# ooowedyn/InkLayer

Measured on AMD Instinct MI355X. Metric: sketches/sec end-to-end (GroundingDINO+SAM) at 1024x1024, higher is better.
Workload: dtype f16 (MFMA, f32 accumulate; f32 residual/norm/softmax; split-f16 = fp32-grade operands for patch-embed, neck, mask decoder); 1 GPU; full GroundingDINO Swin-T + SAM ViT-H pipeline, batch=8 per GPU, 1024x1024 synthetic sketches, 16 boxes/sketch, random-init weights; global_batch=8, parallelism=image-parallel x1

## Files before the change

include/inklayer_hip.h:

```cpp
#ifndef INKLAYER_HIP_H
#define INKLAYER_HIP_H

#include <stdint.h>

#ifdef __cplusplus
extern "C" {
#endif

#define INK_ABI_VERSION 8
int ink_abi_version(void);

typedef struct InkGemm {
  const void* A;
  const void* W;
  const float* bias;
  const float* col_scale;
  const float* residual;
  const int32_t* row_map;
  void* C;
  int32_t M, N, K;
  int32_t lda, ldw, ldr, ldc;
  int32_t act;
  int32_t c_f16;
} InkGemm;
// ... 119 lines not shown
                     int64_t ldo, void* stream);

int ink_attn_fewq(const void* Q, int64_t ldq, const void* K, int64_t ldk, const void* V, int64_t ldv,
                  int32_t n_batch, int32_t n_q, int32_t n_k, int32_t n_heads, int32_t head_dim, float scale,
                  const int32_t* q_batch_rows, const int32_t* kv_batch_rows, const float* k_add, void* O, int64_t ldo,
                  void* stream);

int ink_biattn_colstats(const float* scores, int32_t B, int32_t S, int32_t HT, float* part_ws, float* stats, void* stream);

int ink_fusion_fold_workspace(int32_t B, int32_t S, int64_t* out_floats);
int ink_fusion_fold(float* v_f32, int32_t B, int32_t S, const float* lnv_g, const float* lnv_b, float eps,
                    const float* text_k_f32, const float* text_vl_f32, int64_t ld_text, int32_t T, const void* Wq_f16,
                    const float* bq, const void* Wvv_f16, const float* bvv, const void* Wo_f16, const float* bo,
                    const float* gamma_v, float scale, float* ws, void* out_l_f16, const float* pos, void* out16_pos,
                    void* out16, void* stream);

int ink_sam_upscale_pack(const void* ws_f16, void* blob_f16, void* stream);
int ink_sam_upscale_tail(const float* u0, int64_t ld_tok, int32_t n, int32_t g, const float* ln_g, const float* ln_b, float eps,
                         const void* blob_f16, const float* b3, const float* hyper, int32_t n_masks, float* low,
                         void* stream);

int ink_proj256_ln_pack(const void* ws_f16, void* blob_f16, void* stream);
int ink_proj256_ln(const float* a_f32, const void* blob_f16, const float* bias, const float* res_f32,
                   const int32_t* res_batch_rows, int32_t rows_per_batch, const float* ln_g, const float* ln_b, float eps,
                   int64_t rows, float* out_f32, void* out_split_f16, void* stream);

int ink_ffn256_pack_bytes(int32_t hid, int32_t with_pre, int64_t* out_bytes);
int ink_ffn256_pack(const void* w1_f16, const float* b1, const void* w2_f16, int32_t hid, const void* wpre_f16, void* blob,
                    void* stream);
int ink_ffn256_fused(const void* x_f16, int64_t ldx, const float* res_f32, const void* blob, const float* b2,
                     const float* ln_g, const float* ln_b, float eps, int32_t M, int32_t hid, const float* pre_bias,
                     const float* pre_ln_g, const float* pre_ln_b, float* out_f32, void* stream);

int ink_topk_rowmax(const float* logits, int32_t B, int32_t S, int32_t T, int32_t K, int32_t* out_idx,
                    float* out_val, void* cand_ws, void* stream);

int ink_sine_embed4(const float* ref, const float* dim_t, int32_t N, void* out_f16, void* stream);

int ink_box_refine(const float* delta, int64_t ldd, const float* ref, int32_t N, int32_t ref_is_logit,
                   float* out, void* stream);

int ink_mask_cleanup_workspace_ints(int32_t n, int32_t H, int32_t W, int32_t k, int64_t* out_ints);
int ink_mask_cleanup(const void* masks_u8, int32_t n, int32_t H, int32_t W, int32_t k, int32_t area_threshold,
                     double aspect_threshold, void* tmp_a_u8, void* tmp_b_u8, int32_t* workspace, void* out_u8,
                     void* stream);

int ink_mask_sketch_iou_counts(const void* masks_u8, const void* sketch_rgb_u8, int32_t n, int32_t H, int32_t W,
                               void* bits_ws_u64, int32_t* counts, void* stream);

int ink_sam_amg_stats(const float* low, int32_t n, const int32_t* index, int32_t m, const int32_t* m_dev, int32_t S,
                      int32_t L, int32_t in_h, int32_t in_w, int32_t crop_h, int32_t crop_w, double thr, double offset,
                      int32_t x0, int32_t y0, int32_t orig_h, int32_t orig_w, int32_t* table, void* planes_u64,
                      float* out_logits, void* stream);

int ink_mask_rle_counts(const void* planes_u64, const int32_t* select, int32_t k, int32_t H, int32_t W,
                        int32_t* n_counts, void* stream);
int ink_mask_rle_write(const void* planes_u64, const int32_t* select, int32_t k, int32_t H, int32_t W,
                       const int32_t* offsets, int32_t* counts, void* stream);

int ink_mask_small_regions_workspace_ints(int32_t k, int32_t H, int32_t W, int64_t* out_ints);
int ink_mask_small_regions(const void* planes_u64, int32_t k, int32_t H, int32_t W, int32_t min_area, int32_t holes,
                           void* tmp_planes_u64, int32_t* workspace, void* out_planes_u64, int32_t* changed, void* stream);

int ink_box_nms(const float* boxes, const float* scores, int32_t n, float iou_threshold, void* workspace_u64,
                int32_t* keep, int32_t* n_keep, void* stream);

// ... 114 lines not shown
```

inklayer_amd/_lib.py:

```python
from __future__ import annotations

import ctypes as C
import os
from pathlib import Path

_LIB_PATH = Path(__file__).resolve().parent / "lib" / "libinklayer_hip.so"
_lib = None

c_void_p, c_int, c_i64, c_float = C.c_void_p, C.c_int32, C.c_int64, C.c_float


class InkGemm(C.Structure):
    _fields_ = [
        ("A", c_void_p), ("W", c_void_p), ("bias", c_void_p), ("col_scale", c_void_p),
        ("residual", c_void_p), ("row_map", c_void_p), ("C", c_void_p),
        ("M", c_int), ("N", c_int), ("K", c_int),
        ("lda", c_int), ("ldw", c_int), ("ldr", c_int), ("ldc", c_int),
        ("act", c_int), ("c_f16", c_int),
    ]


class InkAttn(C.Structure):
    _fields_ = [
        ("Q", c_void_p), ("K", c_void_p), ("V", c_void_p), ("O", c_void_p),
# ... 40 lines not shown
                               c_void_p],
    "ink_box_nms": [c_void_p, c_void_p, c_int, c_float, c_void_p, c_void_p, c_void_p, c_void_p],
    "ink_ms_deform_attn_forward": [c_void_p, C.POINTER(c_i64), C.POINTER(c_i64), c_void_p, c_void_p, c_int,
                                   c_int, c_int, c_int, c_int, c_int, c_int, c_int, c_void_p, c_void_p],
    "ink_ms_deform_attn_forward_dev": [c_void_p, c_void_p, c_void_p, c_void_p, c_void_p, c_int, c_int, c_int, c_int,
                                       c_int, c_int, c_int, c_int, c_int, c_void_p, c_void_p],
    "ink_ms_deform_attn_backward_dev": [c_void_p, c_void_p, c_void_p, c_void_p, c_void_p, c_void_p, c_int, c_int, c_int,
                                        c_int, c_int, c_int, c_int, c_int, c_int, c_void_p, c_void_p, c_void_p,
                                        c_void_p],
    "ink_msda_fused": [c_void_p, c_void_p, c_i64, c_void_p, c_int, c_i64, c_i64, C.POINTER(c_int), c_int,
                       c_int, c_int, c_void_p, c_void_p],
    "ink_swin_patchify": [c_void_p, c_int, c_int, C.POINTER(c_float), C.POINTER(c_float), c_void_p, c_void_p],
    "ink_layernorm_merge4": [c_void_p, c_i64, c_void_p, c_void_p, c_float, c_void_p, c_int, c_int, c_void_p,
                             c_void_p],
    "ink_groupnorm_nhwc": [c_void_p, c_int, c_int, c_int, c_int, c_void_p, c_void_p, c_float, c_void_p,
                           c_void_p, c_i64, c_void_p],
    "ink_gather_rows": [c_void_p, c_i64, c_i64, c_void_p, c_i64, c_int, c_int, c_int, c_void_p, c_void_p,
                        c_void_p],
    "ink_biattn_fusion": [c_void_p, c_void_p, c_int, c_int, c_int, c_int, c_float, c_void_p, c_void_p,
                          c_void_p, c_int, c_void_p, c_void_p, c_void_p],
    "ink_biattn_colstats": [c_void_p, c_int, c_int, c_int, c_void_p, c_void_p, c_void_p],
    "ink_fusion_fold_workspace": [c_int, c_int, C.POINTER(c_i64)],
    "ink_relpos_bias64_f16": [c_void_p, c_i64, c_void_p, c_void_p, c_int, c_int, c_int, c_float, c_void_p, c_void_p, c_void_p],
    "ink_proj256_ln_pack": [c_void_p, c_void_p, c_void_p],
    "ink_proj256_ln": [c_void_p, c_void_p, c_void_p, c_void_p, c_void_p, c_int, c_void_p, c_void_p, c_float, c_i64, c_void_p,
                       c_void_p, c_void_p],
    "ink_sam_upscale_pack": [c_void_p, c_void_p, c_void_p],
    "ink_sam_upscale_tail": [c_void_p, c_i64, c_int, c_int, c_void_p, c_void_p, c_float, c_void_p, c_void_p, c_void_p,
                             c_int, c_void_p, c_void_p],
    "ink_ffn256_pack_bytes": [c_int, c_int, C.POINTER(c_i64)],
    "ink_ffn256_pack": [c_void_p, c_void_p, c_void_p, c_int, c_void_p, c_void_p, c_void_p],
    "ink_ffn256_fused": [c_void_p, c_i64, c_void_p, c_void_p, c_void_p, c_void_p, c_void_p, c_float, c_int, c_int,
                         c_void_p, c_void_p, c_void_p, c_void_p, c_void_p],
    "ink_fusion_fold": [c_void_p, c_int, c_int, c_void_p, c_void_p, c_float, c_void_p, c_void_p, c_i64, c_int, c_void_p,
                        c_void_p, c_void_p, c_void_p, c_void_p, c_void_p, c_void_p, c_float, c_void_p, c_void_p, c_void_p,
                        c_void_p, c_void_p, c_void_p],
    "ink_attn_fewkeys": [c_void_p, c_i64, c_void_p, c_i64, c_void_p, c_i64, c_int, c_int, c_int, c_int, c_int,
                         c_float, c_void_p, c_void_p, c_void_p, c_int, c_void_p, c_i64, c_void_p],
    "ink_attn_fewq": [c_void_p, c_i64, c_void_p, c_i64, c_void_p, c_i64, c_int, c_int, c_int, c_int, c_int,
                      c_float, c_void_p, c_void_p, c_void_p, c_void_p, c_i64, c_void_p],
    "ink_topk_rowmax": [c_void_p, c_int, c_int, c_int, c_int, c_void_p, c_void_p, c_void_p, c_void_p],
    "ink_sine_embed4": [c_void_p, c_void_p, c_int, c_void_p, c_void_p],
    "ink_box_refine": [c_void_p, c_i64, c_void_p, c_int, c_int, c_void_p, c_void_p],
    "ink_mask_cleanup_workspace_ints": [c_int, c_int, c_int, c_int, C.POINTER(c_i64)],
    "ink_mask_cleanup": [c_void_p, c_int, c_int, c_int, c_int, c_int, C.c_double, c_void_p, c_void_p, c_void_p,
                         c_void_p, c_void_p],
    "ink_mask_sketch_iou_counts": [c_void_p, c_void_p, c_int, c_int, c_int, c_void_p, c_void_p, c_void_p],
    "ink_refine_sketch_planes": [c_void_p, c_int, c_int, c_void_p, c_void_p, c_void_p],
    "ink_bitplane_pack": [c_void_p, c_int, c_int, c_int, c_int, c_void_p, c_void_p],
    "ink_refine_depth_samples": [c_void_p, c_int, c_void_p, c_void_p, c_int, c_int, c_int, c_void_p, c_void_p, c_void_p],
    "ink_refine_pair_tables": [c_void_p, c_void_p, c_int, c_int, c_int, c_void_p, c_void_p, c_void_p, c_void_p,
                               c_void_p, c_void_p],
    "ink_refine_composite": [c_void_p, c_void_p, c_int, c_int, c_int, c_void_p, c_void_p, c_void_p],
    "ink_refine_relabel_clean": [c_void_p, c_void_p, c_int, c_int, c_void_p, c_void_p],
    "ink_refine_grow_workspace": [c_int, c_int, C.POINTER(c_i64), C.POINTER(c_i64)],
    "ink_refine_grow": [c_void_p, c_void_p, c_int, c_int, c_void_p, c_void_p, c_void_p, c_void_p, c_void_p, c_void_p,
                        c_int, c_void_p, c_void_p],
    "ink_refine_query_dists": [c_void_p, c_void_p, c_void_p, c_int, c_int, c_int, c_void_p, c_void_p],
    "ink_refine_finalize": [c_void_p, c_void_p, c_int, c_void_p, c_int, c_int, c_void_p, c_void_p, c_void_p, c_void_p],
    "ink_host_sparse_sample": [c_void_p, c_int, c_int, c_void_p, c_int, c_void_p],
    "ink_host_assign_unlabeled": [c_void_p, c_int, c_void_p, c_int, c_void_p, c_void_p, c_void_p, c_int, c_void_p],
    "ink_depth_patchify": [c_void_p, c_int, c_int, c_int, c_int, c_int, c_int, C.POINTER(C.c_double), C.POINTER(C.c_double),
                           c_int, c_void_p, c_void_p],
    "ink_resize_bilinear_ac_nhwc": [c_void_p, c_int, c_int, c_int, c_int, c_int, c_int, c_void_p, c_void_p, c_void_p],
    "ink_im2col3x3_ex_f16": [c_void_p, c_int, c_int, c_int, c_int, c_int, c_int, c_void_p, c_void_p],
    "ink_layers_otsu_planes": [c_void_p, c_int, c_int, c_int, c_int, c_void_p, c_void_p, c_void_p, c_void_p],
# ... 64 lines not shown
```

inklayer_amd/build.py:

```python
from __future__ import annotations

import os
import subprocess
import sys
from concurrent.futures import ThreadPoolExecutor
from pathlib import Path

ROOT = Path(__file__).resolve().parent
CSRC = ROOT / "csrc"
LIBDIR = ROOT / "lib"
OBJDIR = LIBDIR / "obj"
LIB = LIBDIR / "libinklayer_hip.so"
HIPCC = os.environ.get("HIPCC", "/opt/rocm/bin/hipcc")
FLAGS = ["--offload-arch=gfx950", "-O3", "-std=c++17", "-fPIC", "-ffp-contract=off",
         "-mllvm", "-amdgpu-mfma-vgpr-form",

         "-Wall", "-Wno-unused-function", "-Wno-unused-variable"]


def _newest_header() -> float:
    hs = list(CSRC.glob("*.h")) + list((ROOT.parent / "include").glob("*.h"))
    return max(h.stat().st_mtime for h in hs)


NO_SPILL = {"ffn_fused.hip", "proj_ln.hip", "amg.hip", "layers.hip", "inpaint_ops.hip", "visualize.hip"}


def _check_no_spill(src: Path, remarks: str) -> None:
    name = None
    for line in remarks.splitlines():
        if "Function Name:" in line:
            name = line.split("Function Name:")[1].split("[")[0].strip()
        elif "ScratchSize [bytes/lane]:" in line:
            n = int(line.split("ScratchSize [bytes/lane]:")[1].split("[")[0])
            if n != 0:
                raise RuntimeError(f"{src.name}: kernel {name} spills ({n} bytes of scratch per lane) - the kernels of "
                                   f"this file must stay in registers (see NO_SPILL); reduce register pressure")


def _compile(src: Path, force: bool, hdr_time: float) -> Path:
    obj = OBJDIR / (src.stem + ".o")
    if (not force and obj.exists() and obj.stat().st_mtime > src.stat().st_mtime
            and obj.stat().st_mtime > hdr_time):
        return obj
    guard = src.name in NO_SPILL
    cmd = [HIPCC, *FLAGS, *(["-Rpass-analysis=kernel-resource-usage", "-fno-caret-diagnostics"] if guard else []), "-c", str(src), "-o", str(obj)]
    r = subprocess.run(cmd, capture_output=True, text=True)
    if r.returncode != 0:
        raise RuntimeError(f"hipcc failed for {src.name}:\n{r.stdout}\n{r.stderr}")
    err = r.stderr
    if guard:
        try:
            _check_no_spill(src, err)
        except RuntimeError:
            obj.unlink(missing_ok=True)
            raise
        err = "\n".join(l for l in err.splitlines()
                        if "kernel-resource-usage" not in l and not l.startswith("In file included from"))
# ... 28 lines not shown
```

inklayer_amd/gdino.py:

```python
from __future__ import annotations

import math
from dataclasses import dataclass
from typing import Dict, List, Optional, Sequence, Tuple

import numpy as np
import torch

from . import ops
from ._lru import LRU

F16, F32, I32 = torch.float16, torch.float32, torch.int32


@dataclass
class GDinoConfig:
    embed_dim: int = 96
    depths: Tuple[int, ...] = (2, 2, 6, 2)
    num_heads: Tuple[int, ...] = (3, 6, 12, 24)
    window_size: int = 7
    out_indices: Tuple[int, ...] = (1, 2, 3)
    hidden_dim: int = 256
    nheads: int = 8
    enc_layers: int = 6
# ... 137 lines not shown
            refs.append(torch.stack((rx.reshape(-1) / ww, ry.reshape(-1) / hh), -1))
            gy, gx = torch.meshgrid(torch.linspace(0, hh - 1, hh), torch.linspace(0, ww - 1, ww), indexing="ij")
            grid = (torch.stack((gx, gy), -1) + 0.5) / torch.tensor([float(ww), float(hh)])
            props.append(torch.cat((grid, torch.ones_like(grid) * 0.05 * (2.0 ** lvl)), -1).view(-1, 4))
        self.enc_ref = torch.cat(refs, 0).to(dev).contiguous()
        pr = torch.cat(props, 0)
        valid = ((pr > 0.01) & (pr < 0.99)).all(-1)
        pr = torch.log(pr / (1 - pr)).masked_fill(~valid[:, None], float("inf"))
        self.props_unsig = pr.to(dev).contiguous()
        self.valid_map = torch.where(valid, torch.arange(self.S), torch.full((self.S,), -1)).to(I32).to(dev)


def swin_dense_bias(table: torch.Tensor, ws: int, nh: int, scale: float) -> torch.Tensor:
    co = torch.stack(torch.meshgrid(torch.arange(ws), torch.arange(ws), indexing="ij")).flatten(1)
    rel = (co[:, :, None] - co[:, None, :]).permute(1, 2, 0).contiguous()
    rel[:, :, 0] += ws - 1
    rel[:, :, 1] += ws - 1
    rel[:, :, 0] *= 2 * ws - 1
    rel_index = rel.sum(-1).view(-1)
    bias = torch.zeros((nh, ws * ws, 64))
    bias[:, :, :ws * ws] = table[rel_index].view(ws * ws, ws * ws, nh).permute(2, 0, 1) / scale
    return bias


def clean_state_dict(sd: Dict[str, torch.Tensor]) -> Dict[str, torch.Tensor]:
    if any(k.startswith("module.") for k in sd):
        return {(k[7:] if k.startswith("module.") else k): v for k, v in sd.items()}
    return sd


class GDinoEngine:
    fuse_ffn = True
    fuse_ffn_pre = True
    fold_fusion = True

    def __init__(self, state_dict: Dict[str, torch.Tensor], cfg: Optional[GDinoConfig] = None,
                 device: str | torch.device = "cuda", encoded_text: Optional[torch.Tensor] = None,
                 token_ids: Sequence[int] = DEFAULT_TOKEN_IDS):
        cfg = cfg or GDinoConfig()
        self.cfg, self.dev = cfg, torch.device(device)
        assert self.dev.type == "cuda", "the InkLayer detector runs on MI355X only"
        assert cfg.hidden_dim == 256 and cfg.nheads == 8 and cfg.num_feature_levels == 4 and cfg.n_points == 4
        assert all(cfg.embed_dim * 2 ** i // nh == 32 for i, nh in enumerate(cfg.num_heads))
        sd, dev = clean_state_dict(state_dict), self.dev
        self.w: Dict[str, torch.Tensor] = {}
        w = self.w

        def h(name, shape=None):
            t = sd[name].detach().to(torch.float32)
            return (t.reshape(shape) if shape is not None else t).to(dev, F16).contiguous()

        def f(name):
            return ops.own_f32(sd[name], dev)

        def lin(dst, src):
            w[dst + ".w"], w[dst + ".b"] = h(src + ".weight"), f(src + ".bias")

        def ln(dst, src):
            w[dst + ".w"], w[dst + ".b"] = f(src + ".weight"), f(src + ".bias")

        def cat_lin(dst, srcs):
            w[dst + ".w"] = torch.cat([h(s + ".weight") for s in srcs]).contiguous()
            w[dst + ".b"] = torch.cat([f(s + ".bias") for s in srcs]).contiguous()

        bb = "backbone.0."
        pw = sd[bb + "patch_embed.proj.weight"].detach().to(torch.float32).cpu().reshape(cfg.embed_dim, 48)
# ... 38 lines not shown
            W, b = sd[src + "in_proj_weight"].detach().to(torch.float32), sd[src + "in_proj_bias"].detach().to(torch.float32)
            D = W.shape[1]
            w[dst + ".qk.w"], w[dst + ".qk.b"] = W[:2 * D].to(dev, F16).contiguous(), b[:2 * D].to(dev).contiguous()
            w[dst + ".q.w"], w[dst + ".q.b"] = W[:D].to(dev, F16).contiguous(), b[:D].to(dev).contiguous()
            w[dst + ".kv.w"], w[dst + ".kv.b"] = W[D:].to(dev, F16).contiguous(), b[D:].to(dev).contiguous()
            w[dst + ".v.w"], w[dst + ".v.b"] = W[2 * D:].to(dev, F16).contiguous(), b[2 * D:].to(dev).contiguous()
            lin(dst + ".out", src + "out_proj")

        for i in range(cfg.enc_layers):
            p, d = f"{t}encoder.layers.{i}.", f"e{i}"
            msda(d + ".msda", p + "self_attn.")
            ln(d + ".norm1", p + "norm1"); lin(d + ".lin1", p + "linear1"); lin(d + ".lin2", p + "linear2"); ln(d + ".norm2", p + "norm2")
            if w[d + ".lin1.w"].shape[1] == 256 and w[d + ".lin1.w"].shape[0] % 64 == 0 and w[d + ".lin1.w"].shape[0] <= 2048:
                w[d + ".ffn.blob"] = ops.ffn256_pack(w[d + ".lin1.w"], w[d + ".lin1.b"], w[d + ".lin2.w"])
                w[d + ".ffn.blob_pre"] = ops.ffn256_pack(w[d + ".lin1.w"], w[d + ".lin1.b"], w[d + ".lin2.w"],
                                                         w[d + ".msda.out.w"])
            p = f"{t}encoder.text_layers.{i}."
            mha(d + ".txt", p + "self_attn.")
            lin(d + ".txt.lin1", p + "linear1"); lin(d + ".txt.lin2", p + "linear2")
            ln(d + ".txt.norm1", p + "norm1"); ln(d + ".txt.norm2", p + "norm2")
            p = f"{t}encoder.fusion_layers.{i}."
            ln(d + ".fu.lnv", p + "layer_norm_v"); ln(d + ".fu.lnl", p + "layer_norm_l")
            cat_lin(d + ".fu.qv", [p + "attn.v_proj", p + "attn.values_v_proj"])
            cat_lin(d + ".fu.kl", [p + "attn.l_proj", p + "attn.values_l_proj"])
            lin(d + ".fu.outv", p + "attn.out_v_proj"); lin(d + ".fu.outl", p + "attn.out_l_proj")
            w[d + ".fu.gv"], w[d + ".fu.gl"] = f(p + "gamma_v"), f(p + "gamma_l")
        for i in range(cfg.dec_layers):
            p, d = f"{t}decoder.layers.{i}.", f"d{i}"
            msda(d + ".msda", p + "cross_attn.")
            ln(d + ".norm1", p + "norm1")
            mha(d + ".ca", p + "ca_text."); ln(d + ".canorm", p + "catext_norm")
            mha(d + ".sa", p + "self_attn."); ln(d + ".norm2", p + "norm2")
            lin(d + ".lin1", p + "linear1"); lin(d + ".lin2", p + "linear2"); ln(d + ".norm3", p + "norm3")
        ln("dec.norm", t + "decoder.norm")
        lin("rph0", t + "decoder.ref_point_head.layers.0")
        lin("rph1", t + "decoder.ref_point_head.layers.1")
        w["tgt"] = f(t + "tgt_embed.weight")
        lin("enc_output", t + "enc_output"); ln("enc_output_norm", t + "enc_output_norm")
        for j in range(3):
            lin(f"encbox{j}", f"{t}enc_out_bbox_embed.layers.{j}")
            lin(f"box{j}", f"bbox_embed.0.layers.{j}")
        dt = torch.arange(128, dtype=torch.float32)
        w["dim_t"] = (10000 ** (2 * torch.div(dt, 2, rounding_mode="floor") / 128)).to(dev)
        self._graphs = LRU(self.graph_cache_size)
        self._plans = LRU(self.plan_cache_size)
        self._seen: Dict[Tuple[int, int, int], int] = {}
        self.set_text(encoded_text, token_ids)

    def set_text(self, encoded_text: Optional[torch.Tensor], token_ids: Sequence[int]) -> None:
        if encoded_text is None:
            raise ValueError("encoded_text [T,256] is required: fold BERT + feat_map once at load "
                             "(inklayer_amd.text_branch) or pass precomputed features")
        T = encoded_text.shape[0]
        assert T == len(token_ids) and T <= 4, "fusion kernel is specialised for captions of <= 4 tokens"
        self._graphs.clear()
        self._seen.clear()
        self.T = T
        self.text0 = encoded_text.detach().to(self.dev, F32).contiguous()
        sm, pid = text_masks_and_position_ids(list(token_ids))
        self.text_blocked = (~sm).to(torch.uint8).to(self.dev).contiguous()
        dim_t = torch.arange(256, dtype=torch.float32)
        dim_t = 10000.0 ** (2 * torch.div(dim_t, 2, rounding_mode="floor") / 256)
        self.pos_text = _interleaved_sincos(pid.float()[:, None] * (2 * math.pi) / dim_t).to(self.dev).contiguous()

    graph_max_batch = 1
    graph_cache_size = 4
# ... 139 lines not shown
        text = ops.layernorm_rows(ops.gemm(ff, w[d + ".txt.lin2.w"], w[d + ".txt.lin2.b"], residual=text),
                                  w[d + ".txt.norm2.w"], w[d + ".txt.norm2.b"], 1e-5, out_dtype=F32)
        if have16:
            proj = ops.gemm(s16p, w[d + ".msda.proj.w"], w[d + ".msda.proj.b"])
            val = ops.gemm(s16, w[d + ".msda.value.w"], w[d + ".msda.value.b"], out_dtype=F16)
        else:
            proj = ops.gemm(ops.add_cvt_f16(src, pl.pos, out=s16), w[d + ".msda.proj.w"], w[d + ".msda.proj.b"])
            val = ops.gemm(ops.add_cvt_f16(src, out=s16), w[d + ".msda.value.w"], w[d + ".msda.value.b"], out_dtype=F16)
        o = ops.msda_fused(val, proj, pl.enc_ref, pl.shapes, B, S, ref_batched=False)
        if self.fuse_ffn and self.fuse_ffn_pre and (d + ".ffn.blob_pre") in w:
            ops.ffn256_fused(o, src, w[d + ".ffn.blob_pre"], int(w[d + ".lin1.b"].numel()), w[d + ".lin2.b"],
                             w[d + ".norm2.w"], w[d + ".norm2.b"], 1e-5, out=src,
                             pre=(w[d + ".msda.out.b"], w[d + ".norm1.w"], w[d + ".norm1.b"]))
            return src, text
        y = ops.gemm(o, w[d + ".msda.out.w"], w[d + ".msda.out.b"], residual=src, out=src)
        ops.layernorm_rows(y, w[d + ".norm1.w"], w[d + ".norm1.b"], 1e-5, out=src, out2=s16)
        if self.fuse_ffn and (d + ".ffn.blob") in w:
            ops.ffn256_fused(s16, src, w[d + ".ffn.blob"], int(w[d + ".lin1.b"].numel()), w[d + ".lin2.b"],
                             w[d + ".norm2.w"], w[d + ".norm2.b"], 1e-5, out=src)
        else:
            ff = ops.gemm(s16, w[d + ".lin1.w"], w[d + ".lin1.b"], act="relu", out_dtype=F16)
            y = ops.gemm(ff, w[d + ".lin2.w"], w[d + ".lin2.b"], residual=src, out=src)
            ops.layernorm_rows(y, w[d + ".norm2.w"], w[d + ".norm2.b"], 1e-5, out=src)
        return src, text

    def decoder(self, memory: torch.Tensor, text: torch.Tensor, pl: _Plan, B: int, stages: Optional[dict] = None):
        cfg, w, dev, T, S, nq = self.cfg, self.w, self.dev, self.T, pl.S, self.cfg.num_queries
        om16 = ops.gather_rows(memory, pl.valid_map, B, S, x_batch_rows=S, idx_batch_stride=0)
        om = ops.gemm(om16, w["enc_output.w"], w["enc_output.b"])
        omn16 = torch.empty((B * S, 256), device=dev, dtype=F16)
        omn = ops.layernorm_rows(om, w["enc_output_norm.w"], w["enc_output_norm.b"], 1e-5, out=om, out2=omn16)
        text16 = ops.add_cvt_f16(text)
        logits = torch.empty((B, S, T), device=dev, dtype=F32)
        for b in range(B):
            ops.gemm(omn16[b * S:(b + 1) * S], text16[b * T:(b + 1) * T], out=logits[b])
        idx = ops.topk_rowmax(logits, nq)
        if stages is not None:
            stages["topk_logits"] = logits
            if "force_topk" in stages:
                idx = stages["force_topk"].to(I32).to(dev).contiguous()
        sel16 = ops.gather_rows(omn, idx, B, nq, x_batch_rows=S, idx_batch_stride=nq)
        delta = self._mlp3("encbox", sel16)
        prop = ops.gather_rows(pl.props_unsig, idx, B, nq, x_batch_rows=0, idx_batch_stride=nq, out_dtype=F32)
        ref = ops.box_refine(delta, prop, ref_is_logit=True)
        if stages is not None:
            stages["topk"], stages["ref0"] = idx, ref
        output = w["tgt"].repeat(B, 1)
        mem16 = ops.add_cvt_f16(memory)
        hs16 = None
        if stages is not None:
            stages["hs"], stages["refs"] = [], [ref.clone()]
        for i in range(cfg.dec_layers):
            output = self._dec_layer(i, output, ref, mem16, text16, pl, B)
            if stages is not None:
                stages["hs"].append(output.clone())
            if i < cfg.dec_layers - 1:
                ref = ops.box_refine(self._mlp3("box", ops.add_cvt_f16(output)), ref)
                if stages is not None:
                    stages["refs"].append(ref.clone())
            else:
                if stages is not None:
                    stages["refs"].append(ops.box_refine(self._mlp3("box", ops.add_cvt_f16(output)), ref))
                hs16 = ops.layernorm_rows(output, w["dec.norm.w"], w["dec.norm.b"], 1e-5)
        boxes = ops.box_refine(self._mlp3("box", hs16), ref).view(B, nq, 4)
        out_logits = torch.empty((B, nq, T), device=dev, dtype=F32)
        for b in range(B):
            ops.gemm(hs16[b * nq:(b + 1) * nq], text16[b * T:(b + 1) * T], out=out_logits[b])
        return out_logits, boxes

    def _dec_layer(self, i: int, output: torch.Tensor, ref: torch.Tensor, mem16: torch.Tensor, text16: torch.Tensor,
                   pl: _Plan, B: int) -> torch.Tensor:
        w = self.w
        nq = output.shape[0] // B
        d = f"d{i}"
        qse = ops.sine_embed4(ref, w["dim_t"])
        qpos = ops.gemm(ops.gemm(qse, w["rph0.w"], w["rph0.b"], act="relu", out_dtype=F16), w["rph1.w"], w["rph1.b"])
        qk = ops.gemm(ops.add_cvt_f16(output, qpos), w[d + ".sa.qk.w"], w[d + ".sa.qk.b"], out_dtype=F16)
        vv = ops.gemm(ops.add_cvt_f16(output), w[d + ".sa.v.w"], w[d + ".sa.v.b"], out_dtype=F16)
        a = ops.flash_attn(qk[:, :256], qk[:, 256:], vv, n_batch=B, n_heads=8, head_dim=32, scale=32 ** -0.5,
                           n_q=nq, n_k=nq)
        output = ops.layernorm_rows(ops.gemm(a, w[d + ".sa.out.w"], w[d + ".sa.out.b"], residual=output),
                                    w[d + ".norm2.w"], w[d + ".norm2.b"], 1e-5, out_dtype=F32)
        q = ops.gemm(ops.add_cvt_f16(output, qpos), w[d + ".ca.q.w"], w[d + ".ca.q.b"], out_dtype=F16)
        kv = ops.gemm(text16, w[d + ".ca.kv.w"], w[d + ".ca.kv.b"], out_dtype=F16)
        a = ops.attn_fewkeys(q, kv[:, :256], kv[:, 256:], B=B, n_heads=8, head_dim=32, scale=32 ** -0.5)
        output = ops.layernorm_rows(ops.gemm(a, w[d + ".ca.out.w"], w[d + ".ca.out.b"], residual=output),
                                    w[d + ".canorm.w"], w[d + ".canorm.b"], 1e-5, out_dtype=F32)
        proj = ops.gemm(ops.add_cvt_f16(output, qpos), w[d + ".msda.proj.w"], w[d + ".msda.proj.b"])
        val = ops.gemm(mem16, w[d + ".msda.value.w"], w[d + ".msda.value.b"], out_dtype=F16)
        o = ops.msda_fused(val, proj, ref, pl.shapes, B, nq, ref_batched=True)
        output = ops.layernorm_rows(ops.gemm(o, w[d + ".msda.out.w"], w[d + ".msda.out.b"], residual=output),
                                    w[d + ".norm1.w"], w[d + ".norm1.b"], 1e-5, out_dtype=F32)
        ff = ops.gemm(ops.add_cvt_f16(output), w[d + ".lin1.w"], w[d + ".lin1.b"], act="relu", out_dtype=F16)
        output = ops.layernorm_rows(ops.gemm(ff, w[d + ".lin2.w"], w[d + ".lin2.b"], residual=output),
                                    w[d + ".norm3.w"], w[d + ".norm3.b"], 1e-5, out_dtype=F32)
        return output

    def forward(self, images_u8: Sequence[torch.Tensor], stages: Optional[dict] = None, allow_graph: bool = True):
        B = len(images_u8)
        sizes = [tuple(im.shape[:2]) for im in images_u8]
        if len(set(sizes)) > 1:
            assert stages is None
            logits = torch.empty((B, self.cfg.num_queries, self.T), device=self.dev, dtype=F32)
            boxes = torch.empty((B, self.cfg.num_queries, 4), device=self.dev, dtype=F32)
            for sz in dict.fromkeys(sizes):
                idx = [i for i, s_ in enumerate(sizes) if s_ == sz]
                lg, bx = self.forward([images_u8[i] for i in idx], allow_graph=allow_graph)
                ii = torch.tensor(idx, device=self.dev)
                logits[ii] = lg
                boxes[ii] = bx
            return logits, boxes
        h, w_ = sizes[0]
        if allow_graph and stages is None and 0 < B <= self.graph_max_batch:
            return self._forward_graphed(images_u8, h, w_)
        return self._forward_eager(images_u8, stages)

    def _forward_eager(self, images_u8: Sequence[torch.Tensor], stages: Optional[dict] = None):
        B = len(images_u8)
        h, w_ = tuple(images_u8[0].shape[:2])
        pl = self.plan(h, w_, B)
        feats = self.backbone(images_u8, pl)
        src = self.neck(feats, pl, B)
        if stages is not None:
# ... 25 lines not shown
```

inklayer_amd/ops.py:

```python
from __future__ import annotations

import ctypes as C
from typing import Optional, Sequence, Tuple

import torch

from . import _lib
from ._lib import InkAttn, InkGemm, check

ACT = {None: 0, "none": 0, "gelu": 1, "relu": 2}
F16, F32 = torch.float16, torch.float32


_GEMM_TRACE = None


def set_gemm_trace(lst) -> None:
    global _GEMM_TRACE
    _GEMM_TRACE = lst


_ATTN_TRACE = None


# ... 770 lines not shown
    assert tuple(w1.shape) == (hid, 256) and tuple(w2.shape) == (256, hid)
    assert b1.dtype == F32 and b1.is_contiguous() and b1.numel() == hid
    assert w_pre is None or (w_pre.dtype == F16 and w_pre.is_contiguous() and tuple(w_pre.shape) == (256, 256))
    need = C.c_int64(0)
    check(_lib.lib().ink_ffn256_pack_bytes(hid, int(w_pre is not None), C.byref(need)), "ink_ffn256_pack_bytes")
    blob = torch.empty(need.value // 2, device=w1.device, dtype=F16)
    check(_lib.lib().ink_ffn256_pack(w1.data_ptr(), b1.data_ptr(), w2.data_ptr(), hid, _p(w_pre), blob.data_ptr(), _stream()),
          "ink_ffn256_pack")
    return blob


def ffn256_fused(x16: torch.Tensor, res: torch.Tensor, blob: torch.Tensor, hid: int, b2: torch.Tensor,
                 ln_g: torch.Tensor, ln_b: torch.Tensor, eps: float, out: Optional[torch.Tensor] = None,
                 pre: Optional[Tuple[torch.Tensor, torch.Tensor, torch.Tensor]] = None) -> torch.Tensor:
    M = int(x16.shape[0])
    assert x16.dtype == F16 and x16.stride(1) == 1 and x16.shape[1] == 256
    assert res.dtype == F32 and res.is_contiguous() and tuple(res.shape) == (M, 256)
    need = C.c_int64(0)
    check(_lib.lib().ink_ffn256_pack_bytes(hid, int(pre is not None), C.byref(need)), "ink_ffn256_pack_bytes")
    assert blob.dtype == F16 and blob.numel() * 2 == need.value and b2.dtype == F32
    assert b2.numel() == 256 and ln_g.numel() == 256 and ln_b.numel() == 256 and ln_g.dtype == F32 and ln_b.dtype == F32
    if pre is not None:
        assert all(t.dtype == F32 and t.is_contiguous() and t.numel() == 256 for t in pre)
    if out is None:
        out = torch.empty_like(res)
    assert out.dtype == F32 and out.is_contiguous() and tuple(out.shape) == (M, 256)
    pb, pg, pe = pre if pre is not None else (None, None, None)
    check(_lib.lib().ink_ffn256_fused(x16.data_ptr(), x16.stride(0), res.data_ptr(), blob.data_ptr(), b2.data_ptr(),
                                      ln_g.data_ptr(), ln_b.data_ptr(), eps, M, hid, _p(pb), _p(pg), _p(pe), out.data_ptr(),
                                      _stream()), "ink_ffn256_fused")
    return out


def attn_fewkeys(q: torch.Tensor, k: torch.Tensor, v: torch.Tensor, *, B: int, n_heads: int, head_dim: int,
                 scale: float, blocked: Optional[torch.Tensor] = None, n_q: Optional[int] = None,
                 q_batch_rows: Optional[torch.Tensor] = None, q_add: Optional[torch.Tensor] = None) -> torch.Tensor:
    io = q.dtype
    for t in (q, k, v):
        assert t.dtype == io and io in (F16, F32) and t.dim() == 2 and t.stride(1) == 1
        assert t.data_ptr() % 16 == 0
    if n_q is None:
        n_q = q.shape[0] // B
    n_k = k.shape[0] // B
    out = torch.empty((B * n_q, n_heads * head_dim), device=q.device, dtype=io)
    if blocked is not None:
        assert blocked.dtype == torch.uint8 and blocked.is_contiguous() and blocked.shape == (n_q, n_k)
    if q_batch_rows is not None:
        assert q_batch_rows.dtype == torch.int32 and q_batch_rows.numel() == B and q_batch_rows.is_cuda
    if q_add is not None:
        assert q_add.dtype == F32 and q_add.is_contiguous() and tuple(q_add.shape) == (n_q, n_heads * head_dim)
    check(_lib.lib().ink_attn_fewkeys(q.data_ptr(), q.stride(0), k.data_ptr(), k.stride(0), v.data_ptr(),
                                      v.stride(0), B, n_q, n_k, n_heads, head_dim, scale, _p(blocked),
                                      _p(q_batch_rows), _p(q_add), int(io == F32), out.data_ptr(), out.stride(0), _stream()),
          "ink_attn_fewkeys")
    return out


def attn_fewq(q: torch.Tensor, k: torch.Tensor, v: torch.Tensor, *, n_batch: int, n_heads: int, head_dim: int,
              scale: float, n_q: int, n_k: int, q_batch_rows: Optional[torch.Tensor] = None,
              kv_batch_rows: Optional[torch.Tensor] = None, k_add: Optional[torch.Tensor] = None) -> torch.Tensor:
    for t in (q, k, v):
        assert t.dtype == F32 and t.dim() == 2 and t.stride(1) == 1
        assert t.data_ptr() % 16 == 0
    for rows in (q_batch_rows, kv_batch_rows):
        assert rows is None or (rows.dtype == torch.int32 and rows.numel() == n_batch and rows.is_cuda)
    out = torch.empty((n_batch * n_q, n_heads * head_dim), device=q.device, dtype=F32)
# ... 393 lines not shown
```

Before: 117.9 sketches/s.

## Fuse GroundingDINO decoder out-proj+residual+LayerNorm rows and batch text logits

Adds a rowchain256 kernel that fuses the 256x256 attention output projection with bias, residual add, LayerNorm, and the f16 conversion of output+qpos into one launch. It replaces the GEMM, layernorm and add_cvt sequence after both self-attention and cross-attention in each decoder layer. The decoder MSDA output projection and FFN tail now go through the existing fused ffn256 kernel with the pre-projection folded in. A batched text-logits kernel replaces per-batch GEMM loops when T<=4. The aim is fewer launches and less intermediate traffic in this latency-bound decoder, at the cost of new hand-scheduled MFMA/LDS code that is pinned to one wave per EU.

```diff
diff --git a/include/inklayer_hip.h b/include/inklayer_hip.h
--- a/include/inklayer_hip.h
+++ b/include/inklayer_hip.h
@@ -175,6 +175,14 @@
                      const float* ln_g, const float* ln_b, float eps, int32_t M, int32_t hid, const float* pre_bias,
                      const float* pre_ln_g, const float* pre_ln_b, float* out_f32, void* stream);
 
+int ink_rows_text_logits(const void* x_f16, const void* text_f16, int32_t B, int32_t rows, int32_t T, float* out_f32,
+                         void* stream);
+
+int ink_rowchain256_pack(const void* w_f16, void* blob_f16, void* stream);
+int ink_rowchain256(const void* x_f16, int64_t ldx, const void* blob_f16, const float* bias, const float* res_f32,
+                    const float* ln_g, const float* ln_b, float eps, int32_t rows, const float* addend_f32, float* out_f32,
+                    void* out_f16, void* out_add_f16, void* stream);
+
 int ink_topk_rowmax(const float* logits, int32_t B, int32_t S, int32_t T, int32_t K, int32_t* out_idx,
                     float* out_val, void* cand_ws, void* stream);
 
diff --git a/inklayer_amd/_lib.py b/inklayer_amd/_lib.py
--- a/inklayer_amd/_lib.py
+++ b/inklayer_amd/_lib.py
@@ -96,6 +96,10 @@
     "ink_ffn256_pack": [c_void_p, c_void_p, c_void_p, c_int, c_void_p, c_void_p, c_void_p],
     "ink_ffn256_fused": [c_void_p, c_i64, c_void_p, c_void_p, c_void_p, c_void_p, c_void_p, c_float, c_int, c_int,
                          c_void_p, c_void_p, c_void_p, c_void_p, c_void_p],
+    "ink_rows_text_logits": [c_void_p, c_void_p, c_int, c_int, c_int, c_void_p, c_void_p],
+    "ink_rowchain256_pack": [c_void_p, c_void_p, c_void_p],
+    "ink_rowchain256": [c_void_p, c_i64, c_void_p, c_void_p, c_void_p, c_void_p, c_void_p, c_float, c_int, c_void_p,
+                        c_void_p, c_void_p, c_void_p, c_void_p],
     "ink_fusion_fold": [c_void_p, c_int, c_int, c_void_p, c_void_p, c_float, c_void_p, c_void_p, c_i64, c_int, c_void_p,
                         c_void_p, c_void_p, c_void_p, c_void_p, c_void_p, c_void_p, c_float, c_void_p, c_void_p, c_void_p,
                         c_void_p, c_void_p, c_void_p],
diff --git a/inklayer_amd/build.py b/inklayer_amd/build.py
--- a/inklayer_amd/build.py
+++ b/inklayer_amd/build.py
@@ -23,7 +23,7 @@
     return max(h.stat().st_mtime for h in hs)
 
 
-NO_SPILL = {"ffn_fused.hip", "proj_ln.hip", "amg.hip", "layers.hip", "inpaint_ops.hip", "visualize.hip"}
+NO_SPILL = {"ffn_fused.hip", "proj_ln.hip", "detector_rows.hip", "amg.hip", "layers.hip", "inpaint_ops.hip", "visualize.hip"}
 
 
 def _check_no_spill(src: Path, remarks: str) -> None:
diff --git a/inklayer_amd/csrc/detector_rows.hip b/inklayer_amd/csrc/detector_rows.hip
--- /dev/null
+++ b/inklayer_amd/csrc/detector_rows.hip
@@ -0,0 +1,265 @@
+#include <type_traits>
+#include "common.h"
+#include "../../include/inklayer_hip.h"
+
+namespace {
+
+typedef __attribute__((address_space(1))) const void* gptr_t;
+typedef __attribute__((address_space(3))) void* lptr_t;
+typedef __attribute__((address_space(3))) char* lds_char_ptr;
+
+constexpr int D = 256, TMAX = 4;
+
+__global__ __launch_bounds__(256) void rows_text_logits_kernel(const f16* __restrict__ x, const f16* __restrict__ text,
+                                                               int rows, int T, float* __restrict__ out) {
+  const int b = blockIdx.y, lane = threadIdx.x & 63, wave = threadIdx.x >> 6;
+  const int sub = lane & 31, half = lane >> 5;
+  float ts[TMAX][8];
+#pragma unroll
+  for (int t = 0; t < TMAX; ++t) {
+    const f16x8 v = *(const f16x8*)(text + ((int64_t)b * T + min(t, T - 1)) * D + sub * 8);
+#pragma unroll
+    for (int j = 0; j < 8; ++j) ts[t][j] = (float)v[j];
+  }
+  const int r0 = blockIdx.x * 64 + wave * 16;
+#pragma unroll 2
+  for (int i = 0; i < 8; ++i) {
+    const int r = r0 + 2 * i + half;
+    const f16x8 v = *(const f16x8*)(x + ((int64_t)b * rows + min(r, rows - 1)) * D + sub * 8);
+    float acc[TMAX];
+#pragma unroll
+    for (int t = 0; t < TMAX; ++t) {
+      float a = 0.f;
+#pragma unroll
+      for (int j = 0; j < 8; ++j) a = fmaf((float)v[j], ts[t][j], a);
+#pragma unroll
+      for (int o = 1; o < 32; o <<= 1) a += __shfl_xor(a, o, 64);
+      acc[t] = a;
+    }
+    if (sub == 0 && r < rows)
+      for (int t = 0; t < T; ++t) out[((int64_t)b * rows + r) * T + t] = acc[t];
+  }
+}
+
+constexpr int C = 256, BM = 128;
+constexpr int BLK = 1024;
+constexpr int NSEG = 2, KSEG = 8;
+constexpr int NBLK = (C / 32) * KSEG;
+constexpr int CHUNK = NBLK * BLK;
+constexpr int PAR_BYTES = 3 * C * 4;
+constexpr int OROW = C * 4 + 16;
+constexpr int PAR_OFF = 4 * 32 * OROW;
+constexpr int LDS_BYTES = PAR_OFF + PAR_BYTES;
+constexpr int DEPTH = 4;
+static_assert(PAR_OFF >= 2 * CHUNK && LDS_BYTES <= 160 * 1024, "LDS layout");
+
+template <int I> using ic = std::integral_constant<int, I>;
+template <int I, int N, class F>
+__device__ __forceinline__ void static_for(F&& f) {
+  if constexpr (I < N) {
+    f(ic<I>{});
+    static_for<I + 1, N>(f);
+  }
+}
+__device__ __forceinline__ f32x16 mfma32(const f16x8& a, const f16x8& b, const f32x16& c) {
+  return __builtin_amdgcn_mfma_f32_32x32x16_f16(a, b, c, 0, 0, 0);
+}
+template <int OFF>
+__device__ __forceinline__ f16x8 lds_frag(uint32_t addr) {
+  f16x8 v;
+  asm volatile("ds_read_b128 %0, %1 offset:%2" : "=v"(v) : "v"(addr), "n"(OFF));
+  return v;
+}
+template <int N>
+__device__ __forceinline__ void wait_frag(f16x8& f) {
+  asm volatile("s_waitcnt lgkmcnt(%1)" : "+v"(f) : "n"(N));
+}
+template <int OFF>
+__device__ __forceinline__ f32x4 lds_f4(uint32_t addr) {
+  f32x4 v;
+  asm volatile("ds_read_b128 %0, %1 offset:%2" : "=v"(v) : "v"(addr), "n"(OFF));
+  return v;
+}
+__device__ __forceinline__ void wait_f4(f32x4& a, f32x4& b, f32x4& c, f32x4& d) {
+  asm volatile("s_waitcnt lgkmcnt(0)" : "+v"(a), "+v"(b), "+v"(c), "+v"(d));
+}
+
+__global__ __launch_bounds__(256) void rowchain_pack_kernel(const f16* __restrict__ W, f16* __restrict__ blob) {
+  const int idx = blockIdx.x * 256 + threadIdx.x;
+  if (idx >= NSEG * NBLK * 64) return;
+  const int lane = idx & 63, q = (idx >> 6) % NBLK, seg = (idx >> 6) / NBLK;
+  const int nt = q / KSEG, s = KSEG * seg + q % KSEG;
+  *(f16x8*)(blob + (int64_t)idx * 8) = *(const f16x8*)(W + (int64_t)(32 * nt + (lane & 31)) * C + 16 * s + 8 * (lane >> 5));
+}
+
+__global__ __launch_bounds__(256) __attribute__((amdgpu_waves_per_eu(1, 1)))
+void rowchain256_kernel(const f16* __restrict__ X, int64_t ldx, const f16* __restrict__ blob, const float* __restrict__ bias,
+                        const float* __restrict__ res, const float* __restrict__ ln_g, const float* __restrict__ ln_b,
+                        float eps, int R, const float* __restrict__ addend, float* __restrict__ out_f32,
+                        f16* __restrict__ out16, f16* __restrict__ out16_add) {
+  extern __shared__ __attribute__((aligned(16))) char smem[];
+  asm volatile("v_accvgpr_write_b32 a255, %0" ::"v"(0) : "a255");
+  const int tid = threadIdx.x, lane = tid & 63;
+  const int wave = __builtin_amdgcn_readfirstlane(tid >> 6);
+  const int l = lane & 31, hh = lane >> 5;
+  const int m0 = blockIdx.x * BM + wave * 32;
+  const int row = min(m0 + l, R - 1);
+  {
+    float* sP = (float*)(smem + PAR_OFF);
+    sP[tid] = bias[tid];
+    sP[C + tid] = ln_g[tid];
+    sP[2 * C + tid] = ln_b[tid];
+  }
+  f16x8 xf[NSEG * KSEG];
+  {
+    const f16* xp = X + (int64_t)row * ldx + 8 * hh;
+#pragma unroll
+    for (int s = 0; s < NSEG * KSEG; ++s) xf[s] = *(const f16x8*)(xp + 16 * s);
+  }
+  f32x16 y[C / 32];
+  {
+    const float* rp = res + (int64_t)row * C + 4 * hh;
+#pragma unroll
+    for (int nt = 0; nt < C / 32; ++nt)
+#pragma unroll
+      for (int g = 0; g < 4; ++g) {
+        const f32x4 r4 = *(const f32x4*)(rp + 32 * nt + 8 * g);
+#pragma unroll
+        for (int e = 0; e < 4; ++e) y[nt][4 * g + e] = r4[e];
+      }
+  }
+  __syncthreads();
+  asm volatile("s_waitcnt vmcnt(0)" ::: "memory");
+
+  auto stage = [&](int buf, int seg, int k) {
+    const int q = 4 * k + wave;
+    __builtin_amdgcn_global_load_lds((gptr_t)((const char*)blob + (int64_t)seg * CHUNK + q * BLK + lane * 16),
+                                     (lptr_t)(smem + buf * CHUNK + q * BLK), 16, 0, 0);
+  };
+#pragma unroll
+  for (int k = 0; k < NBLK / 4; ++k) stage(0, 0, k);
+  const uint32_t lds0 = (uint32_t)(uintptr_t)(lds_char_ptr)smem + lane * 16;
+  const uint32_t par0 = (uint32_t)(uintptr_t)(lds_char_ptr)smem + PAR_OFF + 16 * hh;
+
+  static_for<0, NSEG>([&](auto cc) {
+    constexpr int seg = decltype(cc)::value;
+    asm volatile("s_waitcnt vmcnt(0)" ::: "memory");
+    __builtin_amdgcn_s_barrier();
+    asm volatile("" ::: "memory");
+    const uint32_t wa = lds0 + (seg & 1) * CHUNK;
+    f16x8 fr[DEPTH + 1];
+    auto read = [&](auto ii) {
+      constexpr int i = decltype(ii)::value;
+      fr[i % (DEPTH + 1)] = lds_frag<i * BLK>(wa);
+    };
+    static_for<0, DEPTH>(read);
+    static_for<0, NBLK>([&](auto ii) {
+      constexpr int i = decltype(ii)::value;
+      if constexpr (i + DEPTH < NBLK) read(ic<i + DEPTH>{});
+      wait_frag<(NBLK - 1 - i < DEPTH ? NBLK - 1 - i : DEPTH)>(fr[i % (DEPTH + 1)]);
+      y[i / KSEG] = mfma32(fr[i % (DEPTH + 1)], xf[KSEG * seg + i % KSEG], y[i / KSEG]);
+      if constexpr (seg + 1 < NSEG && i % 4 == 1) stage((seg + 1) & 1, seg + 1, i / 4);
+    });
+  });
+
+  static_for<0, C / 32>([&](auto ii) {
+    constexpr int nt = decltype(ii)::value;
+    constexpr int ob = (32 * nt) * 4;
+    f32x4 c0 = lds_f4<ob>(par0), c1 = lds_f4<ob + 32>(par0), c2 = lds_f4<ob + 64>(par0), c3 = lds_f4<ob + 96>(par0);
+    wait_f4(c0, c1, c2, c3);
+#pragma unroll
+    for (int e = 0; e < 4; ++e) {
+      y[nt][e] += c0[e];
+      y[nt][4 + e] += c1[e];
+      y[nt][8 + e] += c2[e];
+      y[nt][12 + e] += c3[e];
+    }
+  });
+  float sum = 0.f;
+#pragma unroll
+  for (int nt = 0; nt < C / 32; ++nt)
+#pragma unroll
+    for (int r = 0; r < 16; ++r) sum += y[nt][r];
+  sum += __shfl_xor(sum, 32, 64);
+  const float mean = sum * (1.0f / C);
+  float sq = 0.f;
+#pragma unroll
+  for (int nt = 0; nt < C / 32; ++nt)
+#pragma unroll
+    for (int r = 0; r < 16; ++r) {
+      const float d = y[nt][r] - mean;
+      sq += d * d;
+    }
+  sq += __shfl_xor(sq, 32, 64);
+  const float rstd = 1.0f / sqrtf(sq * (1.0f / C) + eps);
+  __syncthreads();
+  char* ot = smem + wave * 32 * OROW;
+  static_for<0, C / 32 * 2>([&](auto ii) {
+    constexpr int nt = decltype(ii)::value / 2, g = 2 * (decltype(ii)::value % 2);
+    constexpr int o0 = C * 4 + (32 * nt + 8 * g) * 4;
+    f32x4 g0 = lds_f4<o0>(par0), g1 = lds_f4<o0 + 32>(par0), b0 = lds_f4<C * 4 + o0>(par0), b1 = lds_f4<C * 4 + o0 + 32>(par0);
+    wait_f4(g0, g1, b0, b1);
+    f32x4 v0, v1;
+#pragma unroll
+    for (int e = 0; e < 4; ++e) {
+      v0[e] = (y[nt][4 * g + e] - mean) * rstd * g0[e] + b0[e];
+      v1[e] = (y[nt][4 * g + 4 + e] - mean) * rstd * g1[e] + b1[e];
+    }
+    *(f32x4*)(ot + l * OROW + (32 * nt + 8 * g + 4 * hh) * 4) = v0;
+    *(f32x4*)(ot + l * OROW + (32 * nt + 8 * g + 8 + 4 * hh) * 4) = v1;
+  });
+#pragma unroll 2
+  for (int r = 0; r < 32; ++r) {
+    const int m = m0 + r;
+    if (m >= R) break;
+    const f32x4 v = *(const f32x4*)(ot + r * OROW + lane * 16);
+    *(f32x4*)(out_f32 + (int64_t)m * C + lane * 4) = v;
+    if (out16) {
+      f16x4 h;
+#pragma unroll
+      for (int e = 0; e < 4; ++e) h[e] = (f16)v[e];
+      *(f16x4*)(out16 + (int64_t)m * C + lane * 4) = h;
+    }
+    if (out16_add) {
+      const f32x4 a = *(const f32x4*)(addend + (int64_t)m * C + lane * 4);
+      f16x4 h;
+#pragma unroll
+      for (int e = 0; e < 4; ++e) h[e] = (f16)(v[e] + a[e]);
+      *(f16x4*)(out16_add + (int64_t)m * C + lane * 4) = h;
+    }
+  }
+}
+
+}
+
+extern "C" int ink_rows_text_logits(const void* x_f16, const void* text_f16, int32_t B, int32_t rows, int32_t T,
+                                    float* out_f32, void* stream) {
+  INK_CHECK_ARG(x_f16 && text_f16 && out_f32 && B > 0 && B < 65536 && rows > 0 && T > 0 && T <= TMAX);
+  INK_CHECK_ARG((((uintptr_t)x_f16 | (uintptr_t)text_f16) & 15) == 0);
+  hipLaunchKernelGGL(rows_text_logits_kernel, dim3((unsigned)((rows + 63) / 64), (unsigned)B), dim3(256), 0,
+                     (hipStream_t)stream, (const f16*)x_f16, (const f16*)text_f16, rows, T, out_f32);
+  return ink_launch_status();
+}
+
+extern "C" int ink_rowchain256_pack(const void* w_f16, void* blob_f16, void* stream) {
+  INK_CHECK_ARG(w_f16 && blob_f16 && ((((uintptr_t)w_f16 | (uintptr_t)blob_f16) & 15) == 0));
+  hipLaunchKernelGGL(rowchain_pack_kernel, dim3((NSEG * NBLK * 64 + 255) / 256), dim3(256), 0, (hipStream_t)stream,
+                     (const f16*)w_f16, (f16*)blob_f16);
+  return ink_launch_status();
+}
+
+extern "C" int ink_rowchain256(const void* x_f16, int64_t ldx, const void* blob_f16, const float* bias, const float* res_f32,
+                               const float* ln_g, const float* ln_b, float eps, int32_t rows, const float* addend_f32,
+                               float* out_f32, void* out_f16, void* out_add_f16, void* stream) {
+  INK_CHECK_ARG(x_f16 && blob_f16 && bias && res_f32 && ln_g && ln_b && out_f32 && rows > 0);
+  INK_CHECK_ARG(ldx >= C && ldx % 8 == 0 && (!out_add_f16 || addend_f32) && rows <= (1 << 30));
+  INK_CHECK_ARG((((uintptr_t)x_f16 | (uintptr_t)blob_f16 | (uintptr_t)res_f32 | (uintptr_t)out_f32 | (uintptr_t)out_f16 |
+                  (uintptr_t)out_add_f16 | (uintptr_t)addend_f32) & 15) == 0);
+  static bool attr = ((void)hipFuncSetAttribute((const void*)rowchain256_kernel, hipFuncAttributeMaxDynamicSharedMemorySize,
+                                                LDS_BYTES), true);
+  (void)attr;
+  hipLaunchKernelGGL(rowchain256_kernel, dim3((unsigned)((rows + BM - 1) / BM)), dim3(256), LDS_BYTES, (hipStream_t)stream,
+                     (const f16*)x_f16, ldx, (const f16*)blob_f16, bias, res_f32, ln_g, ln_b, eps, rows, addend_f32, out_f32,
+                     (f16*)out_f16, (f16*)out_add_f16);
+  return ink_launch_status();
+}
diff --git a/inklayer_amd/gdino.py b/inklayer_amd/gdino.py
--- a/inklayer_amd/gdino.py
+++ b/inklayer_amd/gdino.py
@@ -193,6 +193,9 @@
 class GDinoEngine:
     fuse_ffn = True
     fuse_ffn_pre = True
+    fuse_dec_rows = True
+    fuse_dec_tail = True
+    batch_logits = True
     fold_fusion = True
 
     def __init__(self, state_dict: Dict[str, torch.Tensor], cfg: Optional[GDinoConfig] = None,
@@ -297,6 +300,11 @@
             mha(d + ".ca", p + "ca_text."); ln(d + ".canorm", p + "catext_norm")
             mha(d + ".sa", p + "self_attn."); ln(d + ".norm2", p + "norm2")
             lin(d + ".lin1", p + "linear1"); lin(d + ".lin2", p + "linear2"); ln(d + ".norm3", p + "norm3")
+            w[d + ".sa.out.blob"] = ops.rowchain256_pack(w[d + ".sa.out.w"])
+            w[d + ".ca.out.blob"] = ops.rowchain256_pack(w[d + ".ca.out.w"])
+            if w[d + ".lin1.w"].shape[1] == 256 and w[d + ".lin1.w"].shape[0] % 64 == 0 and w[d + ".lin1.w"].shape[0] <= 2048:
+                w[d + ".ffn.blob_pre"] = ops.ffn256_pack(w[d + ".lin1.w"], w[d + ".lin1.b"], w[d + ".lin2.w"],
+                                                         w[d + ".msda.out.w"])
         ln("dec.norm", t + "decoder.norm")
         lin("rph0", t + "decoder.ref_point_head.layers.0")
         lin("rph1", t + "decoder.ref_point_head.layers.1")
@@ -502,8 +510,11 @@
         omn = ops.layernorm_rows(om, w["enc_output_norm.w"], w["enc_output_norm.b"], 1e-5, out=om, out2=omn16)
         text16 = ops.add_cvt_f16(text)
         logits = torch.empty((B, S, T), device=dev, dtype=F32)
-        for b in range(B):
-            ops.gemm(omn16[b * S:(b + 1) * S], text16[b * T:(b + 1) * T], out=logits[b])
+        if self.batch_logits and T <= 4:
+            ops.rows_text_logits(omn16, text16, B, T, out=logits)
+        else:
+            for b in range(B):
+                ops.gemm(omn16[b * S:(b + 1) * S], text16[b * T:(b + 1) * T], out=logits[b])
         idx = ops.topk_rowmax(logits, nq)
         if stages is not None:
             stages["topk_logits"] = logits
@@ -534,8 +545,11 @@
                 hs16 = ops.layernorm_rows(output, w["dec.norm.w"], w["dec.norm.b"], 1e-5)
         boxes = ops.box_refine(self._mlp3("box", hs16), ref).view(B, nq, 4)
         out_logits = torch.empty((B, nq, T), device=dev, dtype=F32)
-        for b in range(B):
-            ops.gemm(hs16[b * nq:(b + 1) * nq], text16[b * T:(b + 1) * T], out=out_logits[b])
+        if self.batch_logits and T <= 4:
+            ops.rows_text_logits(hs16, text16, B, T, out=out_logits)
+        else:
+            for b in range(B):
+                ops.gemm(hs16[b * nq:(b + 1) * nq], text16[b * T:(b + 1) * T], out=out_logits[b])
         return out_logits, boxes
 
     def _dec_layer(self, i: int, output: torch.Tensor, ref: torch.Tensor, mem16: torch.Tensor, text16: torch.Tensor,
@@ -549,16 +563,30 @@
         vv = ops.gemm(ops.add_cvt_f16(output), w[d + ".sa.v.w"], w[d + ".sa.v.b"], out_dtype=F16)
         a = ops.flash_attn(qk[:, :256], qk[:, 256:], vv, n_batch=B, n_heads=8, head_dim=32, scale=32 ** -0.5,
                            n_q=nq, n_k=nq)
-        output = ops.layernorm_rows(ops.gemm(a, w[d + ".sa.out.w"], w[d + ".sa.out.b"], residual=output),
-                                    w[d + ".norm2.w"], w[d + ".norm2.b"], 1e-5, out_dtype=F32)
-        q = ops.gemm(ops.add_cvt_f16(output, qpos), w[d + ".ca.q.w"], w[d + ".ca.q.b"], out_dtype=F16)
+        if self.fuse_dec_rows:
+            output, _, o16p = ops.rowchain256(a, w[d + ".sa.out.blob"], w[d + ".sa.out.b"], output, w[d + ".norm2.w"],
+                                              w[d + ".norm2.b"], 1e-5, addend=qpos, want16_add=True)
+        else:
+            output = ops.layernorm_rows(ops.gemm(a, w[d + ".sa.out.w"], w[d + ".sa.out.b"], residual=output),
+                                        w[d + ".norm2.w"], w[d + ".norm2.b"], 1e-5, out_dtype=F32)
+            o16p = ops.add_cvt_f16(output, qpos)
+        q = ops.gemm(o16p, w[d + ".ca.q.w"], w[d + ".ca.q.b"], out_dtype=F16)
         kv = ops.gemm(text16, w[d + ".ca.kv.w"], w[d + ".ca.kv.b"], out_dtype=F16)
         a = ops.attn_fewkeys(q, kv[:, :256], kv[:, 256:], B=B, n_heads=8, head_dim=32, scale=32 ** -0.5)
-        output = ops.layernorm_rows(ops.gemm(a, w[d + ".ca.out.w"], w[d + ".ca.out.b"], residual=output),
-                                    w[d + ".canorm.w"], w[d + ".canorm.b"], 1e-5, out_dtype=F32)
-        proj = ops.gemm(ops.add_cvt_f16(output, qpos), w[d + ".msda.proj.w"], w[d + ".msda.proj.b"])
+        if self.fuse_dec_rows:
+            output, _, o16p = ops.rowchain256(a, w[d + ".ca.out.blob"], w[d + ".ca.out.b"], output, w[d + ".canorm.w"],
+                                              w[d + ".canorm.b"], 1e-5, addend=qpos, want16_add=True)
+        else:
+            output = ops.layernorm_rows(ops.gemm(a, w[d + ".ca.out.w"], w[d + ".ca.out.b"], residual=output),
+                                        w[d + ".canorm.w"], w[d + ".canorm.b"], 1e-5, out_dtype=F32)
+            o16p = ops.add_cvt_f16(output, qpos)
+        proj = ops.gemm(o16p, w[d + ".msda.proj.w"], w[d + ".msda.proj.b"])
         val = ops.gemm(mem16, w[d + ".msda.value.w"], w[d + ".msda.value.b"], out_dtype=F16)
         o = ops.msda_fused(val, proj, ref, pl.shapes, B, nq, ref_batched=True)
+        if self.fuse_dec_tail and (d + ".ffn.blob_pre") in w:
+            return ops.ffn256_fused(o, output, w[d + ".ffn.blob_pre"], int(w[d + ".lin1.b"].numel()), w[d + ".lin2.b"],
+                                    w[d + ".norm3.w"], w[d + ".norm3.b"], 1e-5,
+                                    pre=(w[d + ".msda.out.b"], w[d + ".norm1.w"], w[d + ".norm1.b"]))
         output = ops.layernorm_rows(ops.gemm(o, w[d + ".msda.out.w"], w[d + ".msda.out.b"], residual=output),
                                     w[d + ".norm1.w"], w[d + ".norm1.b"], 1e-5, out_dtype=F32)
         ff = ops.gemm(ops.add_cvt_f16(output), w[d + ".lin1.w"], w[d + ".lin1.b"], act="relu", out_dtype=F16)
diff --git a/inklayer_amd/ops.py b/inklayer_amd/ops.py
--- a/inklayer_amd/ops.py
+++ b/inklayer_amd/ops.py
@@ -826,6 +826,44 @@
     return out
 
 
+def rows_text_logits(x16: torch.Tensor, text16: torch.Tensor, B: int, T: int, out: Optional[torch.Tensor] = None) -> torch.Tensor:
+    assert x16.dtype == F16 and x16.is_contiguous() and x16.shape[1] == 256 and x16.shape[0] % B == 0
+    assert text16.dtype == F16 and text16.is_contiguous() and tuple(text16.shape) == (B * T, 256) and 0 < T <= 4
+    rows = x16.shape[0] // B
+    if out is None:
+        out = torch.empty((B, rows, T), device=x16.device, dtype=F32)
+    assert out.dtype == F32 and out.is_contiguous() and tuple(out.shape) == (B, rows, T)
+    check(_lib.lib().ink_rows_text_logits(x16.data_ptr(), text16.data_ptr(), B, rows, T, out.data_ptr(), _stream()),
+          "ink_rows_text_logits")
+    return out
+
+
+def rowchain256_pack(w16: torch.Tensor) -> torch.Tensor:
+    assert w16.dtype == F16 and w16.is_contiguous() and tuple(w16.shape) == (256, 256)
+    blob = torch.empty(2 * 64 * 64 * 8, device=w16.device, dtype=F16)
+    check(_lib.lib().ink_rowchain256_pack(w16.data_ptr(), blob.data_ptr(), _stream()), "ink_rowchain256_pack")
+    return blob
+
+
+def rowchain256(x16: torch.Tensor, blob: torch.Tensor, bias: torch.Tensor, res: torch.Tensor, ln_g: torch.Tensor,
+                ln_b: torch.Tensor, eps: float, *, addend: Optional[torch.Tensor] = None, want16: bool = False,
+                want16_add: bool = False):
+    R = int(x16.shape[0])
+    assert x16.dtype == F16 and x16.stride(1) == 1 and x16.shape[1] == 256 and x16.stride(0) % 8 == 0
+    assert blob.dtype == F16 and blob.numel() == 2 * 64 * 64 * 8
+    assert res.dtype == F32 and res.is_contiguous() and tuple(res.shape) == (R, 256)
+    assert all(t.dtype == F32 and t.is_contiguous() and t.numel() == 256 for t in (bias, ln_g, ln_b))
+    assert not want16_add or (addend is not None and addend.dtype == F32 and addend.is_contiguous()
+                              and tuple(addend.shape) == (R, 256))
+    of = torch.empty((R, 256), device=x16.device, dtype=F32)
+    o16 = torch.empty((R, 256), device=x16.device, dtype=F16) if want16 else None
+    o16a = torch.empty((R, 256), device=x16.device, dtype=F16) if want16_add else None
+    check(_lib.lib().ink_rowchain256(x16.data_ptr(), x16.stride(0), blob.data_ptr(), bias.data_ptr(), res.data_ptr(),
+                                     ln_g.data_ptr(), ln_b.data_ptr(), eps, R, _p(addend) if want16_add else None,
+                                     of.data_ptr(), _p(o16), _p(o16a), _stream()), "ink_rowchain256")
+    return of, o16, o16a
+
+
 def attn_fewkeys(q: torch.Tensor, k: torch.Tensor, v: torch.Tensor, *, B: int, n_heads: int, head_dim: int,
                  scale: float, blocked: Optional[torch.Tensor] = None, n_q: Optional[int] = None,
                  q_batch_rows: Optional[torch.Tensor] = None, q_add: Optional[torch.Tensor] = None) -> torch.Tensor:
```

Result: no change. 118.2 sketches/s (median of 5 runs) (+0.3%).
